# TejasPote/data_diet_distributed

Measured on AMD Instinct MI355X. Metric: examples scored/sec (whole node), EL2N+GraNd ResNet-18 CIFAR-10, 1/2/4/8 GPU, higher is better.
Workload: dtype fp32 (split MFMA: hi*hi + hi*lo + lo*hi with fp32 accumulation; EL2N forward on f16x3 halves, GraNd forward on f16x3, GraNd backward on bf16x3); 1 GPU; R18/C10 EL2N+GraNd, K checkpoints, global keep-set; arch=resnet18, input=3x32x32 cifar stem, n_examples=50000, checkpoints=10, classes=10, score_batch=128, grand_batch=1024, el2n_chunk=1024, kept=25000, select_by=el2n, pegrad_method=auto, grand_params=conv_linear, passes=sequential, lanes=3, launch_plan=full chunks + short tail, el2n_operands=f16x3

## Files before the change

### data_diet_distributed_amd/csrc/dd_pegrad.hip

```cpp
#include "dd_common.h"
#include "dd_mfma.h"
#include "dd_pgram.h"
#include "dd_stem.h"

namespace dd {

typedef float floatx16 __attribute__((ext_vector_type(16)));
typedef float floatx4 __attribute__((ext_vector_type(4)));

struct Geom {
  int cin, h, w, cout, ho, wo, kh, kw, stride, pad;
};

__device__ __forceinline__ unsigned xcd_remap(unsigned orig, unsigned nwg) {
  const unsigned q = nwg / 8, r = nwg % 8, xcd = orig % 8;
  return (xcd < r ? xcd * (q + 1) : r * (q + 1) + (xcd - r) * q) + orig / 8;
}

constexpr int DBM = 64, DBN = 64, DBK = 32;

__global__ __launch_bounds__(256) void pegrad_direct_kernel(const float* __restrict__ act,
                                                            const float* __restrict__ gout,
                                                            Geom g, int n_cblk, int n_oblk,
                                                            const float* __restrict__ col_scale,
                                                            float* __restrict__ partial) {
  __shared__ float As[DBK][DBM + 1];
  __shared__ float Bs[DBK][DBN + 1];
  __shared__ float red[4];

  const int ntiles = g.kh * g.kw * n_cblk * n_oblk;
  const unsigned lid = xcd_remap(blockIdx.x, gridDim.x);
  const int b = lid / ntiles;
  int tile = lid - b * ntiles;
  const int ob = tile % n_oblk;
  tile /= n_oblk;
  const int cb = tile % n_cblk;
  const int shift = tile / n_cblk;
  const int ky = shift / g.kw, kx = shift - (shift / g.kw) * g.kw;
  const int c0 = cb * DBM, o0 = ob * DBN;
  const int T = g.ho * g.wo, HW = g.h * g.w;
  const float* a_b = act + (size_t)b * g.cin * HW;
  const float* g_b = gout + (size_t)b * g.cout * T;

  const int tid = threadIdx.x, tl = tid & 31, rg = tid >> 5;
  float ra[8], rb[8];
  auto load = [&](int t0) {
    const int t = t0 + tl;
    const bool vt = t < T;
    const int oy = vt ? t / g.wo : 0;
    const int ox = vt ? t - oy * g.wo : 0;
    const int iy = oy * g.stride + ky - g.pad, ix = ox * g.stride + kx - g.pad;
    const bool va = vt && iy >= 0 && iy < g.h && ix >= 0 && ix < g.w;
    const int off = iy * g.w + ix;
#pragma unroll
    for (int j = 0; j < 8; ++j) {
      const int c = c0 + rg + 8 * j;
      ra[j] = (va && c < g.cin) ? a_b[(size_t)c * HW + off] : 0.f;
      const int o = o0 + rg + 8 * j;
      rb[j] = (vt && o < g.cout) ? g_b[(size_t)o * T + t] : 0.f;
    }
  };

  const int lane = tid & 63, wv = tid >> 6, wm = wv & 1, wn = wv >> 1;
  const int kr = lane >> 5, col = lane & 31;
  floatx16 acc = {0};
  const int nk = (T + DBK - 1) / DBK;
  load(0);
  for (int kt = 0; kt < nk; ++kt) {
    __syncthreads();
#pragma unroll
    for (int j = 0; j < 8; ++j) {
      As[tl][rg + 8 * j] = ra[j];
      Bs[tl][rg + 8 * j] = rb[j];
    }
    __syncthreads();
    if (kt + 1 < nk) load((kt + 1) * DBK);
#pragma unroll
    for (int kk = 0; kk < DBK / 2; ++kk) {
      const float av = As[2 * kk + kr][wm * 32 + col];
      const float bv = Bs[2 * kk + kr][wn * 32 + col];
      acc = __builtin_amdgcn_mfma_f32_32x32x2f32(av, bv, acc, 0, 0, 0);
    }
  }
  const int o = o0 + wn * 32 + col;
  float s2 = 1.f;
  if (col_scale) {
    const float s = (o < g.cout) ? col_scale[o] : 0.f;
    s2 = s * s;
  }
  float v = 0.f;
#pragma unroll
  for (int r = 0; r < 16; ++r) v += acc[r] * acc[r];
  v = wave_sum(v * s2);
  if (lane == 0) red[wv] = v;
  __syncthreads();
  if (tid == 0) partial[lid] = (red[0] + red[1]) + (red[2] + red[3]);
}

typedef __bf16 bf16x8_t __attribute__((ext_vector_type(8)));
typedef __bf16 bf16x4_t __attribute__((ext_vector_type(4)));

template <int S, int LC>
__global__ __launch_bounds__(256) void pegrad_direct1x1_kernel(const float* __restrict__ act,
                                                               const float* __restrict__ gout,
                                                               Geom g, int n_cblk, int n_oblk,
                                                               const float* __restrict__ col_scale,
                                                               float* __restrict__ partial) {
  constexpr int LO = 4 / LC;
  constexpr int MC = 64 * LC, MO = 64 * LO, R = MC + MO;
  constexpr int KT = 32;
  constexpr int RS = KT * 2 + 16;
  constexpr int PL = R * RS;
  constexpr int NL = R * (KT / 4) / 256;
  static_assert(R * (KT / 4) % 256 == 0, "whole float4 loads per thread");
  __shared__ __attribute__((aligned(16))) char lds[2 * PL];
  __shared__ float red[4];
  const int ntiles = n_cblk * n_oblk;
  const unsigned lid = xcd_remap(blockIdx.x, gridDim.x);
  const int b = lid / ntiles;
  const int tile = lid - b * ntiles;
  const int ob = tile % n_oblk, cb = tile / n_oblk;
  const int c0 = cb * MC, o0 = ob * MO;
  const int T = g.ho * g.wo, HW = g.h * g.w;
  const int tid = threadIdx.x, lane = tid & 63, wv = tid >> 6;
  const float* __restrict__ a_b = act + (size_t)b * g.cin * HW;
  const float* __restrict__ g_b = gout + (size_t)b * g.cout * T;
  const bool vec = T % 4 == 0 && (S == 1 || g.wo % 4 == 0) && HW % 4 == 0;

  float4 rv[NL];
  auto load = [&](int t0) {
#pragma unroll
    for (int k = 0; k < NL; ++k) {
      const int q = tid + 256 * k, row = q / (KT / 4), x4 = q % (KT / 4);
      const int t = t0 + 4 * x4;
      const bool isa = row < MC;
      const int ch = isa ? c0 + row : o0 + row - MC;
      const bool rok = ch < (isa ? g.cin : g.cout);
      const float* base = isa ? a_b + (size_t)(rok ? ch : 0) * HW
                              : g_b + (size_t)(rok ? ch : 0) * T;
      float v[4] = {0.f, 0.f, 0.f, 0.f};
      if (vec) {
        if (rok && t < T) {
          if (!isa || S == 1) {
            const float4 u = *reinterpret_cast<const float4*>(base + t);
            v[0] = u.x; v[1] = u.y; v[2] = u.z; v[3] = u.w;
          } else {
            const int oy = t / g.wo, ox = t - oy * g.wo;
            const float* src = base + (size_t)oy * S * g.w + ox * S;
            const float4 u0 = *reinterpret_cast<const float4*>(src);
            const float4 u1 = *reinterpret_cast<const float4*>(src + 4);
            v[0] = u0.x; v[1] = u0.z; v[2] = u1.x; v[3] = u1.z;
          }
        }
      } else {
#pragma unroll
        for (int j = 0; j < 4; ++j) {
          const int tj = t + j;
          if (rok && tj < T) {
            int ia = tj;
            if (isa && S != 1) {
              const int oy = tj / g.wo, ox = tj - oy * g.wo;
              ia = oy * S * g.w + ox * S;
            }
            v[j] = base[ia];
          }
        }
      }
      rv[k] = make_float4(v[0], v[1], v[2], v[3]);
    }
  };
  auto stage = [&]() {
#pragma unroll
    for (int k = 0; k < NL; ++k) {
      const int q = tid + 256 * k, row = q / (KT / 4), x4 = q % (KT / 4);
      const float f[4] = {rv[k].x, rv[k].y, rv[k].z, rv[k].w};
      bf16x4_t hv, lv;
#pragma unroll
      for (int j = 0; j < 4; ++j) {
        const __bf16 x = (__bf16)f[j];
        hv[j] = x;
        lv[j] = (__bf16)(f[j] - (float)x);
      }
      char* p = lds + row * RS + x4 * 8;
      *reinterpret_cast<bf16x4_t*>(p) = hv;
      *reinterpret_cast<bf16x4_t*>(p + PL) = lv;
    }
  };

  const int r = lane & 31, h = lane >> 5;
  const int wc = wv % LC, wo_ = wv / LC;
  floatx16 acc[2][2];
#pragma unroll
  for (int i = 0; i < 2; ++i)
#pragma unroll
    for (int j = 0; j < 2; ++j) acc[i][j] = floatx16{0};
  load(0);
  for (int t0 = 0; t0 < T; t0 += KT) {
    __syncthreads();
    stage();
    __syncthreads();
    if (t0 + KT < T) load(t0 + KT);
#pragma unroll
    for (int s = 0; s < 2; ++s) {
      bf16x8_t ah[2], al[2], gh[2], gl[2];
#pragma unroll
      for (int i = 0; i < 2; ++i) {
        const char* pa = lds + (wc * 64 + 32 * i + r) * RS + (16 * s + 8 * h) * 2;
        const char* pg = lds + (MC + wo_ * 64 + 32 * i + r) * RS + (16 * s + 8 * h) * 2;
        ah[i] = *reinterpret_cast<const bf16x8_t*>(pa);
        al[i] = *reinterpret_cast<const bf16x8_t*>(pa + PL);
        gh[i] = *reinterpret_cast<const bf16x8_t*>(pg);
        gl[i] = *reinterpret_cast<const bf16x8_t*>(pg + PL);
      }
#pragma unroll
      for (int i = 0; i < 2; ++i)
#pragma unroll
        for (int j = 0; j < 2; ++j) {
          floatx16 d = acc[i][j];
          d = __builtin_amdgcn_mfma_f32_32x32x16_bf16(ah[i], gh[j], d, 0, 0, 0);
          d = __builtin_amdgcn_mfma_f32_32x32x16_bf16(ah[i], gl[j], d, 0, 0, 0);
          d = __builtin_amdgcn_mfma_f32_32x32x16_bf16(al[i], gh[j], d, 0, 0, 0);
          acc[i][j] = d;
        }
    }
  }
  float v = 0.f;
#pragma unroll
  for (int j = 0; j < 2; ++j) {
    const int o = o0 + wo_ * 64 + 32 * j + r;
    float s2 = 1.f;
    if (col_scale) {
      const float sc = o < g.cout ? col_scale[o] : 0.f;
      s2 = sc * sc;
    }
    float q = 0.f;
#pragma unroll
    for (int i = 0; i < 2; ++i)
#pragma unroll
      for (int k = 0; k < 16; ++k) q += acc[i][j][k] * acc[i][j][k];
    v += q * s2;
  }
  v = wave_sum(v);
  if (lane == 0) red[wv] = v;
  __syncthreads();
  if (tid == 0) partial[lid] = (red[0] + red[1]) + (red[2] + red[3]);
}

__global__ __launch_bounds__(256) void pegrad_ghost64_kernel(const float* __restrict__ act,
                                                             const float* __restrict__ gout,
                                                             Geom g, int nT,
                                                             const float* __restrict__ col_scale,
                                                             float* __restrict__ partial) {
  __shared__ float red[4];
  const int ntiles = nT * nT;
  const unsigned lid = xcd_remap(blockIdx.x, gridDim.x);
  const int b = lid / ntiles;
  const int tile = lid - b * ntiles;
  const int bi = tile / nT, bj = tile - (tile / nT) * nT;
  const int T = g.ho * g.wo, HW = g.h * g.w;
  const float* a_b = act + (size_t)b * g.cin * HW;
  const float* g_b = gout + (size_t)b * g.cout * T;

  const int tid = threadIdx.x, lane = tid & 63, wv = tid >> 6;
  const int h = lane >> 5, r = lane & 31;
  const int ti = bi * 64 + (wv & 1) * 32 + r;
  const int tj = bj * 64 + (wv >> 1) * 32 + r;
  const bool vti = ti < T, vtj = tj < T;
  const int oyi = vti ? ti / g.wo : 0, oxi = vti ? ti - oyi * g.wo : 0;
  const int oyj = vtj ? tj / g.wo : 0, oxj = vtj ? tj - oyj * g.wo : 0;

  floatx16 accA = {0}, accG = {0};
  const int npair = (g.cin + 1) / 2;
  for (int ky = 0; ky < g.kh; ++ky) {
    for (int kx = 0; kx < g.kw; ++kx) {
      const int iyi = oyi * g.stride + ky - g.pad, ixi = oxi * g.stride + kx - g.pad;
      const int iyj = oyj * g.stride + ky - g.pad, ixj = oxj * g.stride + kx - g.pad;
      const bool vi = vti && iyi >= 0 && iyi < g.h && ixi >= 0 && ixi < g.w;
      const bool vj = vtj && iyj >= 0 && iyj < g.h && ixj >= 0 && ixj < g.w;
      const float* pi = a_b + (vi ? iyi * g.w + ixi : 0);
      const float* pj = a_b + (vj ? iyj * g.w + ixj : 0);
      int p = 0;
      for (; p + 4 <= npair; p += 4) {
        float ai[4], aj[4];
#pragma unroll
        for (int u = 0; u < 4; ++u) {
          const int c = 2 * (p + u) + h;
          ai[u] = (vi && c < g.cin) ? pi[(size_t)c * HW] : 0.f;
          aj[u] = (vj && c < g.cin) ? pj[(size_t)c * HW] : 0.f;
        }
#pragma unroll
        for (int u = 0; u < 4; ++u)
          accA = __builtin_amdgcn_mfma_f32_32x32x2f32(ai[u], aj[u], accA, 0, 0, 0);
      }
      for (; p < npair; ++p) {
        const int c = 2 * p + h;
        const float ai = (vi && c < g.cin) ? pi[(size_t)c * HW] : 0.f;
        const float aj = (vj && c < g.cin) ? pj[(size_t)c * HW] : 0.f;
        accA = __builtin_amdgcn_mfma_f32_32x32x2f32(ai, aj, accA, 0, 0, 0);
      }
    }
  }
  const int opair = (g.cout + 1) / 2;
  for (int p = 0; p < opair; ++p) {
    const int o = 2 * p + h;
    const bool vo = o < g.cout;
    const float s = (col_scale && vo) ? col_scale[o] : 1.f;
    const float gi = (vti && vo) ? g_b[(size_t)o * T + ti] * s : 0.f;
    const float gj = (vtj && vo) ? g_b[(size_t)o * T + tj] * s : 0.f;
    accG = __builtin_amdgcn_mfma_f32_32x32x2f32(gi, gj, accG, 0, 0, 0);
  }
  float v = 0.f;
#pragma unroll
  for (int k = 0; k < 16; ++k) v += accA[k] * accG[k];
  v = wave_sum(v);
  if (lane == 0) red[wv] = v;
  __syncthreads();
  if (tid == 0) partial[lid] = (red[0] + red[1]) + (red[2] + red[3]);
}

__global__ __launch_bounds__(256) void pegrad_ghost16_kernel(const float* __restrict__ act,
                                                             const float* __restrict__ gout,
                                                             int64_t B, Geom g,
                                                             const float* __restrict__ col_scale,
                                                             float* __restrict__ partial) {
  const int lane = threadIdx.x & 63;
  const int64_t b = (int64_t)blockIdx.x * 4 + (threadIdx.x >> 6);
  if (b >= B) return;
  const int T = g.ho * g.wo, HW = g.h * g.w;
  const float* a_b = act + (size_t)b * g.cin * HW;
  const float* g_b = gout + (size_t)b * g.cout * T;
  const int t = lane & 15, kq = lane >> 4;
  const bool vt = t < T;
  const int oy = vt ? t / g.wo : 0, ox = vt ? t - oy * g.wo : 0;

  floatx4 a0 = {0}, a1 = {0}, gA = {0}, gB = {0};
  const int nq = (g.cin + 3) / 4;
  for (int ky = 0; ky < g.kh; ++ky) {
    for (int kx = 0; kx < g.kw; ++kx) {
      const int iy = oy * g.stride + ky - g.pad, ix = ox * g.stride + kx - g.pad;
      const bool v = vt && iy >= 0 && iy < g.h && ix >= 0 && ix < g.w;
      const float* p = a_b + (v ? iy * g.w + ix : 0);
      int q = 0;
      for (; q + 4 <= nq; q += 4) {
        float x[4];
#pragma unroll
        for (int u = 0; u < 4; ++u) {
          const int c = 4 * (q + u) + kq;
          x[u] = (v && c < g.cin) ? p[(size_t)c * HW] : 0.f;
        }
        a0 = __builtin_amdgcn_mfma_f32_16x16x4f32(x[0], x[0], a0, 0, 0, 0);
        a1 = __builtin_amdgcn_mfma_f32_16x16x4f32(x[1], x[1], a1, 0, 0, 0);
        a0 = __builtin_amdgcn_mfma_f32_16x16x4f32(x[2], x[2], a0, 0, 0, 0);
        a1 = __builtin_amdgcn_mfma_f32_16x16x4f32(x[3], x[3], a1, 0, 0, 0);
      }
      for (; q < nq; ++q) {
        const int c = 4 * q + kq;
        const float x = (v && c < g.cin) ? p[(size_t)c * HW] : 0.f;
        a0 = __builtin_amdgcn_mfma_f32_16x16x4f32(x, x, a0, 0, 0, 0);
      }
    }
  }
  const int no = (g.cout + 3) / 4;
  int q = 0;
  for (; q + 2 <= no; q += 2) {
    float x[2];
#pragma unroll
    for (int u = 0; u < 2; ++u) {
      const int o = 4 * (q + u) + kq;
      const bool vo = o < g.cout;
      const float s = (col_scale && vo) ? col_scale[o] : 1.f;
      x[u] = (vt && vo) ? g_b[(size_t)o * T + t] * s : 0.f;
    }
    gA = __builtin_amdgcn_mfma_f32_16x16x4f32(x[0], x[0], gA, 0, 0, 0);
    gB = __builtin_amdgcn_mfma_f32_16x16x4f32(x[1], x[1], gB, 0, 0, 0);
  }
  for (; q < no; ++q) {
    const int o = 4 * q + kq;
    const bool vo = o < g.cout;
    const float s = (col_scale && vo) ? col_scale[o] : 1.f;
    const float x = (vt && vo) ? g_b[(size_t)o * T + t] * s : 0.f;
    gA = __builtin_amdgcn_mfma_f32_16x16x4f32(x, x, gA, 0, 0, 0);
  }
  float v = 0.f;
#pragma unroll
  for (int k = 0; k < 4; ++k) v += (a0[k] + a1[k]) * (gA[k] + gB[k]);
  v = wave_sum(v);
  if (lane == 0) partial[b] = v;
}

typedef __bf16 bf16x8 __attribute__((ext_vector_type(8)));
typedef __bf16 bf16x4 __attribute__((ext_vector_type(4)));

template <int W, int STR>
struct D3Cfg {
  static constexpr int R = 32 / W;
  static constexpr int NEW = STR * R;
  static constexpr int WIN = STR == 1 ? R + 2 : 2 * R + 1;
  static constexpr int S = WIN + NEW;
  static constexpr int WI = STR * W;
  static constexpr int CS = ((W * 2 / 16) % 2 == 1 || STR == 2) ? W * 2 : W * 2 + 16;
  static constexpr int PLANE = 64 * CS;
  static constexpr int ACT_BYTES = S * 3 * 2 * PLANE;
  static constexpr int GCS = 80;
  static constexpr int GPLANE = 64 * GCS;
  static constexpr int G_BYTES = 2 * 2 * GPLANE;
  static constexpr int LDS = ACT_BYTES + G_BYTES;
  static constexpr int TPR = WI / 4;
  static constexpr int NA = NEW * 64 * WI / 4 / 256;
  static_assert(NEW * 64 * WI / 4 % 256 == 0, "whole float4 rounds");
  static_assert(LDS <= 160 * 1024, "LDS budget");
};

__device__ __forceinline__ void split4(float4 v, bf16x4& hi, bf16x4& lo) {
  const __bf16 h0 = (__bf16)v.x, h1 = (__bf16)v.y, h2 = (__bf16)v.z, h3 = (__bf16)v.w;
  hi = bf16x4{h0, h1, h2, h3};
  lo = bf16x4{(__bf16)(v.x - (float)h0), (__bf16)(v.y - (float)h1), (__bf16)(v.z - (float)h2),
              (__bf16)(v.w - (float)h3)};
}

template <int W, int STR>
__global__ __launch_bounds__(256, 1) void pegrad_direct3x3_kernel(
    const float* __restrict__ act, const float* __restrict__ gout, int cin, int cout, int H,
    int n_cblk, int n_oblk, const float* __restrict__ col_scale, float* __restrict__ partial) {
  using C = D3Cfg<W, STR>;
  extern __shared__ __attribute__((aligned(16))) char smem[];
  char* act_lds = smem;
  char* g_lds = smem + C::ACT_BYTES;

  const unsigned lid = xcd_remap(blockIdx.x, gridDim.x);
  const int per_ex = n_cblk * n_oblk;
  const int b = lid / per_ex;
  const int rem = lid - b * per_ex;
  const int c0 = (rem / n_oblk) * 64, o0 = (rem % n_oblk) * 64;
  const int HW = H * W;
  const int HI = STR * H, HWI = HI * C::WI;
  const float* a_b = act + (size_t)b * cin * HWI;
  const float* g_b = gout + (size_t)b * cout * HW;

  constexpr int NTH = 256;
  const int tid = threadIdx.x, lane = tid & 63, wv = tid >> 6;
  const int wc = wv & 1, wo = (wv >> 1) & 1, r = lane & 31, h = lane >> 5;

  constexpr int NAT = C::NA, NGT = 2;
  float4 ra[NAT], rg[NGT];
  bool va[NAT], vg[NGT];
  auto load_rows = [&](int ir0, int nrows, int tstep) {
#pragma unroll
    for (int k = 0; k < NAT; ++k) {
      const int idx = tid + NTH * k;
      const int x4 = idx % C::TPR, c = (idx / C::TPR) % 64, rr = idx / (C::TPR * 64);
      const int ir = ir0 + rr;
      const int cg = c0 + c;
      va[k] = rr < nrows && ir >= 0 && ir < HI && cg < cin;
      const int irc = ir < 0 ? 0 : (ir >= HI ? HI - 1 : ir);
      const int cgc = cg < cin ? cg : cin - 1;
      ra[k] = *reinterpret_cast<const float4*>(a_b + (size_t)cgc * HWI + irc * C::WI + x4 * 4);
    }
    if (tstep >= 0) {
      const int ts = tstep < HW / 32 ? tstep : HW / 32 - 1;
#pragma unroll
      for (int k = 0; k < NGT; ++k) {
        const int idx = tid + NTH * k;
        const int o = idx >> 3, t4 = idx & 7;
        const int og = o0 + o;
        vg[k] = og < cout;
        const int ogc = og < cout ? og : cout - 1;
        rg[k] = *reinterpret_cast<const float4*>(g_b + (size_t)ogc * HW + ts * 32 + t4 * 4);
      }
    }
  };
  auto zero_if = [](float4 v, bool ok) { return conv::keep_if(v, ok); };
  auto store_rows = [&](int ir0, int nrows, int gbuf) {
#pragma unroll
    for (int k = 0; k < NAT; ++k) {
      const int idx = tid + NTH * k;
      const int x4 = idx % C::TPR, c = (idx / C::TPR) % 64, rr = idx / (C::TPR * 64);
      if (nrows < C::NEW && rr >= nrows) continue;
      const int slot = (ir0 + rr + 1) % C::S;
      const float4 v = zero_if(ra[k], va[k]);
      if constexpr (STR == 1) {
        static_assert(C::TPR <= 16 && 16 % C::TPR == 0, "row of lanes inside a DPP row");
        uint2 hs[3], ls[3];
        conv::split_shift3(v, x4 == 0, x4 == C::TPR - 1, hs, ls);
#pragma unroll
        for (int kx = 0; kx < 3; ++kx) {
          char* base = act_lds + ((slot * 3 + kx) * 2) * C::PLANE + c * C::CS + x4 * 8;
          *reinterpret_cast<uint2*>(base) = hs[kx];
          *reinterpret_cast<uint2*>(base + C::PLANE) = ls[kx];
        }
      } else {
        float left = conv::lane_prev<C::TPR>(v.w);
        if (x4 == 0) left = 0.f;
        const float f[5] = {left, v.x, v.y, v.z, v.w};
        __bf16 hv[5], lv[5];
#pragma unroll
        for (int i = 0; i < 5; ++i) {
          hv[i] = (__bf16)f[i];
          lv[i] = (__bf16)(f[i] - (float)hv[i]);
        }
        typedef __bf16 bf16x2 __attribute__((ext_vector_type(2)));
#pragma unroll
        for (int kx = 0; kx < 3; ++kx) {
          char* base = act_lds + ((slot * 3 + kx) * 2) * C::PLANE + c * C::CS + x4 * 4;
          *reinterpret_cast<bf16x2*>(base) = bf16x2{hv[kx], hv[kx + 2]};
          *reinterpret_cast<bf16x2*>(base + C::PLANE) = bf16x2{lv[kx], lv[kx + 2]};
        }
      }
    }
    if (gbuf >= 0) {
#pragma unroll
      for (int k = 0; k < NGT; ++k) {
        const int idx = tid + NTH * k;
        const int o = idx >> 3, t4 = idx & 7;
        bf16x4 hi, lo;
        split4(zero_if(rg[k], vg[k]), hi, lo);
        char* base = g_lds + ((gbuf * 2) * 64 + o) * C::GCS + t4 * 8;
        *reinterpret_cast<bf16x4*>(base) = hi;
        *reinterpret_cast<bf16x4*>(base + C::GPLANE) = lo;
      }
    }
  };

  constexpr int NTAP = 9;
  floatx16 acc[NTAP];
#pragma unroll
  for (int i = 0; i < NTAP; ++i) acc[i] = floatx16{0};

  const int nsteps = H / C::R;
  for (int ir0 = -1; ir0 < C::WIN - 1; ir0 += C::NEW) {
    const int n = C::NEW < C::WIN - 1 - ir0 ? C::NEW : C::WIN - 1 - ir0;
    load_rows(ir0, n, ir0 == -1 ? 0 : -1);
    store_rows(ir0, n, ir0 == -1 ? 0 : -1);
  }
  __syncthreads();

  auto frag = [&](int y0, int gbuf, int s, int t, int lo) -> bf16x8 {
    const int tl = 16 * s + 8 * h;
    const int ro = tl / W, x = tl % W;
    if (t < 0) {
      const char* gb = g_lds + ((gbuf * 2) * 64 + wo * 32 + r) * C::GCS + tl * 2;
      return *reinterpret_cast<const bf16x8*>(gb + lo * C::GPLANE);
    }
    const int ky = t / 3, kx = t % 3;
    const int slot = (STR * (y0 + ro) + ky) % C::S;
    const char* ab = act_lds + ((slot * 3 + kx) * 2) * C::PLANE + (wc * 32 + r) * C::CS + x * 2;
    return *reinterpret_cast<const bf16x8*>(ab + lo * C::PLANE);
  };
  auto tap_step = [&](int y0, int gbuf, int inext) {
    bf16x8 bh0, bl0, ah0[NTAP], al0[NTAP], bh1, bl1, ah1[NTAP], al1[NTAP];
    bh0 = frag(y0, gbuf, 0, -1, 0);
    bl0 = frag(y0, gbuf, 0, -1, 1);
    ah0[0] = frag(y0, gbuf, 0, 0, 0);
    al0[0] = frag(y0, gbuf, 0, 0, 1);
    auto rd = [&](int j) {
      constexpr int J0 = 2 * (NTAP - 1), J1 = J0 + 2, J2 = J1 + 2 * NTAP;
      if (j < J0) {
        if (j & 1) al0[1 + j / 2] = frag(y0, gbuf, 0, 1 + j / 2, 1);
        else ah0[1 + j / 2] = frag(y0, gbuf, 0, 1 + j / 2, 0);
      } else if (j < J1) {
        (j == J0 ? bh1 : bl1) = frag(y0, gbuf, 1, -1, j - J0);
      } else if (j < J2) {
        if ((j - J1) & 1) al1[(j - J1) / 2] = frag(y0, gbuf, 1, (j - J1) / 2, 1);
        else ah1[(j - J1) / 2] = frag(y0, gbuf, 1, (j - J1) / 2, 0);
      }
    };
#pragma unroll
    for (int i = 0; i < NTAP; ++i) {
#pragma unroll
      for (int q = 0; q < 3; ++q) {
        __builtin_amdgcn_sched_barrier(0);
        acc[i] = __builtin_amdgcn_mfma_f32_32x32x16_bf16(q == 2 ? al0[i] : ah0[i],
                                                         q == 1 ? bl0 : bh0, acc[i], 0, 0, 0);
        const int g = 3 * i + q;
        const int j0 = g < NTAP ? 2 * g : NTAP + g, nr = g < NTAP ? 2 : 1;
        rd(j0);
        if (nr == 2) rd(j0 + 1);
      }
    }
    __builtin_amdgcn_sched_barrier(0);
#pragma unroll
    for (int i = 0; i < NTAP; ++i) {
      floatx16 a = acc[i];
      a = __builtin_amdgcn_mfma_f32_32x32x16_bf16(ah1[i], bh1, a, 0, 0, 0);
      a = __builtin_amdgcn_mfma_f32_32x32x16_bf16(ah1[i], bl1, a, 0, 0, 0);
      a = __builtin_amdgcn_mfma_f32_32x32x16_bf16(al1[i], bh1, a, 0, 0, 0);
      acc[i] = a;
    }
    store_rows(inext, C::NEW, gbuf ^ 1);
#pragma unroll
    for (int i = 0; i < 3 * NTAP - 1; ++i) {
      __builtin_amdgcn_sched_group_barrier(0x008, 1, 1);
      __builtin_amdgcn_sched_group_barrier(0x002, 4, 1);
      __builtin_amdgcn_sched_group_barrier(0x080, 1, 1);
    }
    __builtin_amdgcn_sched_group_barrier(0x008, 1, 1);
    __builtin_amdgcn_sched_barrier(0);
  };
  for (int st = 0; st < nsteps; ++st) {
    const int y0 = st * C::R;
    const int inext = STR * y0 + C::WIN - 1;
    load_rows(inext, C::NEW, st + 1);
    const int gbuf = st & 1;
    tap_step(y0, gbuf, inext);
    __syncthreads();
  }

  const int o = o0 + wo * 32 + r;
  float s2 = (o < cout) ? 1.f : 0.f;
  if (col_scale && o < cout) {
    const float sc = col_scale[o];
    s2 = sc * sc;
  }
  float v = 0.f;
#pragma unroll
  for (int i = 0; i < NTAP; ++i)
#pragma unroll
    for (int k = 0; k < 16; ++k) v += acc[i][k] * acc[i][k];
  v = wave_sum(v * s2);
  float* red = reinterpret_cast<float*>(smem);
  if (lane == 0) red[wv] = v;
  __syncthreads();
  if (tid == 0) partial[lid] = (red[0] + red[1]) + (red[2] + red[3]);
}

template <int W, int STR>
static void launch_direct3x3(const float* act, const float* gout, int64_t B, int cin, int cout,
                             int H, const float* col_scale, float* partial, hipStream_t st) {
  using C = D3Cfg<W, STR>;
  const int ncb = (int)ceil_div(cin, 64), nob = (int)ceil_div(cout, 64);
  static bool attr_set = false;
  if (!attr_set) {
    (void)hipFuncSetAttribute(reinterpret_cast<const void*>(&pegrad_direct3x3_kernel<W, STR>),
                              hipFuncAttributeMaxDynamicSharedMemorySize, C::LDS);
    attr_set = true;
  }
  pegrad_direct3x3_kernel<W, STR><<<(unsigned)(B * ncb * nob), 256, C::LDS, st>>>(
      act, gout, cin, cout, H, ncb, nob, col_scale, partial);
}

template <int W, int STR>
__global__ __launch_bounds__(256, 1) void pegrad_direct3x3p_kernel(
    const float* __restrict__ act, const float* __restrict__ gout, int cin, int cout, int H,
    int n_cblk, int n_oblk, const float* __restrict__ col_scale, float* __restrict__ partial,
    int total) {
  using C = D3Cfg<W, STR>;
  extern __shared__ __attribute__((aligned(16))) char smem[];
  char* act_lds = smem;
  char* g_lds = smem + C::ACT_BYTES;
  float* red = reinterpret_cast<float*>(smem + C::LDS);

  const int per_ex = n_cblk * n_oblk;
  const int HW = H * W;
  const int HI = STR * H, HWI = HI * C::WI;
  int lid, c0, o0;
  const float *a_b, *g_b;
  auto set_tile = [&](int t) {
    lid = (int)xcd_remap((unsigned)t, (unsigned)total);
    const int b = lid / per_ex;
    const int rem = lid - b * per_ex;
    c0 = (rem / n_oblk) * 64;
    o0 = (rem % n_oblk) * 64;
    a_b = act + (size_t)b * cin * HWI;
    g_b = gout + (size_t)b * cout * HW;
  };

  constexpr int NTH = 256;
  const int tid = threadIdx.x, lane = tid & 63, wv = tid >> 6;
  const int wc = wv & 1, wo = (wv >> 1) & 1, r = lane & 31, h = lane >> 5;

  constexpr int NAW = C::WIN * 64 * C::WI / 4 / NTH;
  static_assert(C::WIN * 64 * C::WI / 4 % NTH == 0, "whole float4 rounds");
  constexpr int NGT = 2;
  float4 ra[NAW], rg[NGT];
  bool va[NAW], vg[NGT];
  auto load_rows = [&](auto NKc, int ir0, int nrows, int tstep) {
    constexpr int NK = decltype(NKc)::value;
#pragma unroll
    for (int k = 0; k < NK; ++k) {
      const int idx = tid + NTH * k;
      const int x4 = idx % C::TPR, c = (idx / C::TPR) % 64, rr = idx / (C::TPR * 64);
      const int ir = ir0 + rr;
      const int cg = c0 + c;
      va[k] = rr < nrows && ir >= 0 && ir < HI && cg < cin;
      const int irc = ir < 0 ? 0 : (ir >= HI ? HI - 1 : ir);
      const int cgc = cg < cin ? cg : cin - 1;
      ra[k] = *reinterpret_cast<const float4*>(a_b + (size_t)cgc * HWI + irc * C::WI + x4 * 4);
    }
    if (tstep >= 0) {
      const int ts = tstep < HW / 32 ? tstep : HW / 32 - 1;
#pragma unroll
      for (int k = 0; k < NGT; ++k) {
        const int idx = tid + NTH * k;
        const int o = idx >> 3, t4 = idx & 7;
        const int og = o0 + o;
        vg[k] = og < cout;
        const int ogc = og < cout ? og : cout - 1;
        rg[k] = *reinterpret_cast<const float4*>(g_b + (size_t)ogc * HW + ts * 32 + t4 * 4);
      }
    }
  };
  auto zero_if = [](float4 v, bool ok) { return conv::keep_if(v, ok); };
  auto store_rows = [&](auto NKc, int ir0, int gbuf) {
    constexpr int NK = decltype(NKc)::value;
#pragma unroll
    for (int k = 0; k < NK; ++k) {
      const int idx = tid + NTH * k;
      const int x4 = idx % C::TPR, c = (idx / C::TPR) % 64, rr = idx / (C::TPR * 64);
      const int slot = (ir0 + rr + 1) % C::S;
      const float4 v = zero_if(ra[k], va[k]);
      if constexpr (STR == 1) {
        static_assert(C::TPR <= 16 && 16 % C::TPR == 0, "row of lanes inside a DPP row");
        uint2 hs[3], ls[3];
        conv::split_shift3(v, x4 == 0, x4 == C::TPR - 1, hs, ls);
#pragma unroll
        for (int kx = 0; kx < 3; ++kx) {
          char* base = act_lds + ((slot * 3 + kx) * 2) * C::PLANE + c * C::CS + x4 * 8;
          *reinterpret_cast<uint2*>(base) = hs[kx];
          *reinterpret_cast<uint2*>(base + C::PLANE) = ls[kx];
        }
      } else {
        float left = conv::lane_prev<C::TPR>(v.w);
        if (x4 == 0) left = 0.f;
        const float f[5] = {left, v.x, v.y, v.z, v.w};
        __bf16 hv[5], lv[5];
#pragma unroll
        for (int i = 0; i < 5; ++i) {
          hv[i] = (__bf16)f[i];
          lv[i] = (__bf16)(f[i] - (float)hv[i]);
        }
        typedef __bf16 bf16x2 __attribute__((ext_vector_type(2)));
#pragma unroll
        for (int kx = 0; kx < 3; ++kx) {
          char* base = act_lds + ((slot * 3 + kx) * 2) * C::PLANE + c * C::CS + x4 * 4;
          *reinterpret_cast<bf16x2*>(base) = bf16x2{hv[kx], hv[kx + 2]};
          *reinterpret_cast<bf16x2*>(base + C::PLANE) = bf16x2{lv[kx], lv[kx + 2]};
        }
      }
    }
    if (gbuf >= 0) {
#pragma unroll
      for (int k = 0; k < NGT; ++k) {
        const int idx = tid + NTH * k;
        const int o = idx >> 3, t4 = idx & 7;
        bf16x4 hi, lo;
        split4(zero_if(rg[k], vg[k]), hi, lo);
        char* base = g_lds + ((gbuf * 2) * 64 + o) * C::GCS + t4 * 8;
        *reinterpret_cast<bf16x4*>(base) = hi;
        *reinterpret_cast<bf16x4*>(base + C::GPLANE) = lo;
      }
    }
  };

  constexpr int NTAP = 9;
  floatx16 acc[NTAP];
  const std::integral_constant<int, C::NA> KN;
  const std::integral_constant<int, NAW> KW;

  const int nsteps = H / C::R;
  int t = blockIdx.x;
  set_tile(t);
  load_rows(KW, -1, C::WIN, 0);
  store_rows(KW, -1, 0);
  __syncthreads();

  auto frag = [&](int y0, int gbuf, int s, int t, int lo) -> bf16x8 {
    const int tl = 16 * s + 8 * h;
    const int ro = tl / W, x = tl % W;
    if (t < 0) {
      const char* gb = g_lds + ((gbuf * 2) * 64 + wo * 32 + r) * C::GCS + tl * 2;
      return *reinterpret_cast<const bf16x8*>(gb + lo * C::GPLANE);
    }
    const int ky = t / 3, kx = t % 3;
    const int slot = (STR * (y0 + ro) + ky) % C::S;
    const char* ab = act_lds + ((slot * 3 + kx) * 2) * C::PLANE + (wc * 32 + r) * C::CS + x * 2;
    return *reinterpret_cast<const bf16x8*>(ab + lo * C::PLANE);
  };
  auto step = [&](int st, auto LASTc, bool has_next) {
    constexpr bool LAST = decltype(LASTc)::value;
    const int y0 = st * C::R;
    const int inext = STR * y0 + C::WIN - 1;
    if constexpr (!LAST) {
      load_rows(KN, inext, C::NEW, st + 1);
    } else {
      if (has_next) load_rows(KW, -1, C::WIN, 0);
    }
    const int gbuf = st & 1;
    {
      bf16x8 bh0, bl0, ah0[NTAP], al0[NTAP], bh1, bl1, ah1[NTAP], al1[NTAP];
      bh0 = frag(y0, gbuf, 0, -1, 0);
      bl0 = frag(y0, gbuf, 0, -1, 1);
      ah0[0] = frag(y0, gbuf, 0, 0, 0);
      al0[0] = frag(y0, gbuf, 0, 0, 1);
      auto rd = [&](int j) {
        constexpr int J0 = 2 * (NTAP - 1), J1 = J0 + 2, J2 = J1 + 2 * NTAP;
        if (j < J0) {
          if (j & 1) al0[1 + j / 2] = frag(y0, gbuf, 0, 1 + j / 2, 1);
          else ah0[1 + j / 2] = frag(y0, gbuf, 0, 1 + j / 2, 0);
        } else if (j < J1) {
          (j == J0 ? bh1 : bl1) = frag(y0, gbuf, 1, -1, j - J0);
        } else if (j < J2) {
          if ((j - J1) & 1) al1[(j - J1) / 2] = frag(y0, gbuf, 1, (j - J1) / 2, 1);
          else ah1[(j - J1) / 2] = frag(y0, gbuf, 1, (j - J1) / 2, 0);
        }
      };
#pragma unroll
      for (int i = 0; i < NTAP; ++i) {
#pragma unroll
        for (int q = 0; q < 3; ++q) {
          __builtin_amdgcn_sched_barrier(0);
          acc[i] = __builtin_amdgcn_mfma_f32_32x32x16_bf16(q == 2 ? al0[i] : ah0[i],
                                                           q == 1 ? bl0 : bh0, acc[i], 0, 0, 0);
          const int g = 3 * i + q;
          const int j0 = g < NTAP ? 2 * g : NTAP + g, nr = g < NTAP ? 2 : 1;
          rd(j0);
          if (nr == 2) rd(j0 + 1);
        }
      }
      __builtin_amdgcn_sched_barrier(0);
#pragma unroll
      for (int i = 0; i < NTAP; ++i) {
        floatx16 a = acc[i];
        a = __builtin_amdgcn_mfma_f32_32x32x16_bf16(ah1[i], bh1, a, 0, 0, 0);
        a = __builtin_amdgcn_mfma_f32_32x32x16_bf16(ah1[i], bl1, a, 0, 0, 0);
        a = __builtin_amdgcn_mfma_f32_32x32x16_bf16(al1[i], bh1, a, 0, 0, 0);
        acc[i] = a;
      }
      if constexpr (!LAST) {
        store_rows(KN, inext, gbuf ^ 1);
#pragma unroll
        for (int i = 0; i < 3 * NTAP - 1; ++i) {
          __builtin_amdgcn_sched_group_barrier(0x008, 1, 1);
          __builtin_amdgcn_sched_group_barrier(0x002, 4, 1);
          __builtin_amdgcn_sched_group_barrier(0x080, 1, 1);
        }
        __builtin_amdgcn_sched_group_barrier(0x008, 1, 1);
      }
      __builtin_amdgcn_sched_barrier(0);
    }
    __syncthreads();
  };

  for (;;) {
#pragma unroll
    for (int i = 0; i < NTAP; ++i) acc[i] = floatx16{0};
    for (int st = 0; st + 1 < nsteps; ++st) step(st, std::false_type{}, false);
    const int lid_c = lid, o0_c = o0;
    const int tn = t + (int)gridDim.x;
    const bool has_next = tn < total;
    if (has_next) set_tile(tn);
    step(nsteps - 1, std::true_type{}, has_next);

    const int o = o0_c + wo * 32 + r;
    float s2 = (o < cout) ? 1.f : 0.f;
    if (col_scale && o < cout) {
      const float sc = col_scale[o];
      s2 = sc * sc;
    }
    float v = 0.f;
#pragma unroll
    for (int i = 0; i < NTAP; ++i)
#pragma unroll
      for (int k = 0; k < 16; ++k) v += acc[i][k] * acc[i][k];
    v = wave_sum(v * s2);
    if (lane == 0) red[wv] = v;
    if (has_next) store_rows(KW, -1, 0);
    __syncthreads();
    if (tid == 0) partial[lid_c] = (red[0] + red[1]) + (red[2] + red[3]);
    if (!has_next) break;
    __syncthreads();
    t = tn;
  }
}

template <int W, int STR>
static void launch_direct3x3p(const float* act, const float* gout, int64_t B, int cin, int cout,
                              int H, const float* col_scale, float* partial, hipStream_t st) {
  using C = D3Cfg<W, STR>;
  const int ncb = (int)ceil_div(cin, 64), nob = (int)ceil_div(cout, 64);
  constexpr int LDS = C::LDS + 16;
  static_assert(LDS <= 160 * 1024, "LDS budget");
  static bool attr_set = false;
  if (!attr_set) {
    (void)hipFuncSetAttribute(reinterpret_cast<const void*>(&pegrad_direct3x3p_kernel<W, STR>),
                              hipFuncAttributeMaxDynamicSharedMemorySize, LDS);
    attr_set = true;
  }
  const int64_t total = B * ncb * nob;
  const int64_t grid = std::min<int64_t>(total, device_cus());
  pegrad_direct3x3p_kernel<W, STR><<<(unsigned)grid, 256, LDS, st>>>(
      act, gout, cin, cout, H, ncb, nob, col_scale, partial, (int)total);
}

static bool direct3x3_ok(const dd_conv_geom* g) {
  if (g->kh != 3 || g->kw != 3 || g->pad != 1) return false;
  if (g->stride == 1)
    return g->ho == g->h && g->wo == g->w && (g->w == 8 || g->w == 16 || g->w == 32) &&
           (g->h % (32 / g->w)) == 0;
  return g->stride == 2 && g->h == 2 * g->ho && g->w == 2 * g->wo && g->wo == 16 &&
         (g->ho % 2) == 0;
}

__global__ __launch_bounds__(256) void reduce_partials_kernel(const float* __restrict__ partial,
                                                              int64_t B, int ntiles,
                                                              float* __restrict__ sq) {
  const int64_t b = (int64_t)blockIdx.x * blockDim.x + threadIdx.x;
  if (b >= B) return;
  const float* p = partial + b * ntiles;
  float s = 0.f;
  for (int i = 0; i < ntiles; ++i) s += p[i];
  sq[b] += s;
}

struct Plan {
  int method;
  int ghost16;
  int d3x3;
  int d1x1;
  int pgram;
  int pgq;
  int stem;
  int ntiles;
  int n_cblk, n_oblk, nT;
};

static bool geom_ok(const dd_conv_geom* gm) {
  if (!gm) return false;
  if (gm->batch < 0 || gm->cin <= 0 || gm->cout <= 0 || gm->h <= 0 || gm->w <= 0) return false;
  if (gm->kh <= 0 || gm->kw <= 0 || gm->stride <= 0 || gm->pad < 0) return false;
  const int ho = (gm->h + 2 * gm->pad - gm->kh) / gm->stride + 1;
  const int wo = (gm->w + 2 * gm->pad - gm->kw) / gm->stride + 1;
  return ho == gm->ho && wo == gm->wo && ho > 0 && wo > 0;
}

static double direct_cost(const dd_conv_geom* gm) {
  const double T = (double)ceil_div((int64_t)gm->ho * gm->wo, DBK) * DBK;
  const double da = (double)gm->kh * gm->kw * ceil_div(gm->cin, DBM) * DBM;
  const double dg = (double)ceil_div(gm->cout, DBN) * DBN;
  return 2.0 * T * da * dg;
}

static double ghost_cost(const dd_conv_geom* gm) {
  const int64_t T = (int64_t)gm->ho * gm->wo;
  if (T <= 16) {
    const double da = (double)gm->kh * gm->kw * ceil_div(gm->cin, 4) * 4;
    const double dg = (double)ceil_div(gm->cout, 4) * 4;
    return 2.0 * 256.0 * (da + dg);
  }
  const double Tp = (double)ceil_div(T, 64) * 64;
  const double da = (double)gm->kh * gm->kw * ceil_div(gm->cin, 2) * 2;
  const double dg = (double)ceil_div(gm->cout, 2) * 2;
  return 2.0 * Tp * Tp * (da + dg) * 1.5;
}

static constexpr double kD3x3Weight = 0.25;

static int d1x1_layout(const dd_conv_geom* gm) {
  int best = 0;
  double best_eff = 0.0;
  for (int lc = 1; lc <= 4; lc *= 2) {
    const double pc = (double)ceil_div(gm->cin, 64 * lc) * 64 * lc;
    const double po = (double)ceil_div(gm->cout, 64 * (4 / lc)) * 64 * (4 / lc);
    const double eff = (double)gm->cin * gm->cout / (pc * po);
    if (eff > best_eff + 1e-9) {
      best_eff = eff;
      best = lc;
    }
  }
  return best_eff >= 0.75 ? best : 0;
}

static Plan make_plan(const dd_conv_geom* gm, int method, int precision) {
  Plan p{};
  const bool d3 = precision == DD_PREC_BF16X3 && direct3x3_ok(gm);
  const bool d1 = precision == DD_PREC_BF16X3 && gm->kh == 1 && gm->kw == 1 && gm->pad == 0 &&
                  (gm->stride == 1 || gm->stride == 2) &&
                  gm->ho == (gm->h - 1) / gm->stride + 1 &&
                  gm->wo == (gm->w - 1) / gm->stride + 1 && d1x1_layout(gm) > 0;
  if (precision == DD_PREC_BF16X3 && method != DD_PEGRAD_GHOST && stem_ok(gm)) {
    p.method = DD_PEGRAD_DIRECT;
    p.stem = 1;
    p.ntiles = 1;
    return p;
  }
  if (precision == DD_PREC_BF16X3 && method != DD_PEGRAD_DIRECT && pgram_ok(gm)) {
    p.method = DD_PEGRAD_GHOST;
    p.pgram = 1;
    p.ntiles = 1;
    return p;
  }
  if (precision == DD_PREC_BF16X3 && method != DD_PEGRAD_DIRECT && pgram_q_ok(gm) &&
      (method == DD_PEGRAD_GHOST || pgram_q_auto())) {
    p.method = DD_PEGRAD_GHOST;
    p.pgq = 1;
    p.ntiles = 4;
    return p;
  }
  if (method == DD_PEGRAD_AUTO) {
    const double dc = direct_cost(gm) * (d3 ? kD3x3Weight : 1.0);
    method = ghost_cost(gm) < dc ? DD_PEGRAD_GHOST : DD_PEGRAD_DIRECT;
  }
  p.method = method;
  const int64_t T = (int64_t)gm->ho * gm->wo;
  if (method == DD_PEGRAD_DIRECT && d1) {
    p.d1x1 = d1x1_layout(gm);
    p.n_cblk = (int)ceil_div(gm->cin, 64 * p.d1x1);
    p.n_oblk = (int)ceil_div(gm->cout, 64 * (4 / p.d1x1));
    p.ntiles = p.n_cblk * p.n_oblk;
  } else if (method == DD_PEGRAD_DIRECT && d3) {
    p.d3x3 = 1;
    p.n_cblk = (int)ceil_div(gm->cin, 64);
    p.n_oblk = (int)ceil_div(gm->cout, 64);
    p.ntiles = p.n_cblk * p.n_oblk;
  } else if (method == DD_PEGRAD_DIRECT) {
    p.n_cblk = (int)ceil_div(gm->cin, DBM);
    p.n_oblk = (int)ceil_div(gm->cout, DBN);
    p.ntiles = gm->kh * gm->kw * p.n_cblk * p.n_oblk;
  } else {
    p.ghost16 = T <= 16;
    p.nT = (int)ceil_div(T, 64);
    p.ntiles = p.ghost16 ? 1 : p.nT * p.nT;
  }
  return p;
}

}

using namespace dd;

extern "C" {

static bool prec_ok(int precision) {
  return precision == DD_PREC_FP32 || precision == DD_PREC_BF16X3;
}

int dd_conv_pegrad_method(const dd_conv_geom* geom, int method, int precision) {
  clear_error();
  DD_REQUIRE(geom_ok(geom), "dd_conv_pegrad_method: inconsistent conv geometry");
  DD_REQUIRE(method >= DD_PEGRAD_AUTO && method <= DD_PEGRAD_GHOST, "bad method %d", method);
  DD_REQUIRE(prec_ok(precision), "bad precision %d", precision);
  const Plan p = make_plan(geom, method, precision);
  return p.d3x3 ? DD_PEGRAD_DIRECT3X3 : p.d1x1 ? DD_PEGRAD_DIRECT1X1 : p.pgram ? DD_PEGRAD_PGRAM
         : p.pgq ? DD_PEGRAD_PGRAM_Q : p.stem ? DD_PEGRAD_STEM : p.method;
}

size_t dd_conv_pegrad_workspace_bytes(const dd_conv_geom* geom, int method, int precision) {
  if (!geom_ok(geom) || method < DD_PEGRAD_AUTO || method > DD_PEGRAD_GHOST ||
      !prec_ok(precision))
    return 0;
  const Plan p = make_plan(geom, method, precision);
  return (size_t)geom->batch * p.ntiles * sizeof(float);
}

int dd_conv_pegrad_sqnorm(const float* act, const float* gout, const dd_conv_geom* geom,
                          const float* col_scale, int method, int precision, float* sq_accum,
                          void* workspace, size_t workspace_bytes, void* stream) {
  clear_error();
  DD_REQUIRE(geom_ok(geom), "dd_conv_pegrad_sqnorm: inconsistent conv geometry");
  DD_REQUIRE(method >= DD_PEGRAD_AUTO && method <= DD_PEGRAD_GHOST, "bad method %d", method);
  DD_REQUIRE(prec_ok(precision), "bad precision %d", precision);
  const int64_t B = geom->batch;
  if (B == 0) return DD_OK;
  DD_REQUIRE(act && gout && sq_accum, "dd_conv_pegrad_sqnorm: null buffer");
  DD_REQUIRE((int64_t)geom->cin * geom->h * geom->w < (1ll << 31) &&
                 (int64_t)geom->cout * geom->ho * geom->wo < (1ll << 31),
             "dd_conv_pegrad_sqnorm: per-example tensor too large");
  const Plan p = make_plan(geom, method, precision);
  const size_t need = (size_t)B * p.ntiles * sizeof(float);
  if (workspace_bytes < need || !workspace) {
    set_error("dd_conv_pegrad_sqnorm: workspace %zu < %zu bytes", workspace_bytes, need);
    return DD_EWORKSPACE;
  }
  float* partial = static_cast<float*>(workspace);
  Geom g{geom->cin, geom->h, geom->w, geom->cout, geom->ho, geom->wo,
         geom->kh, geom->kw, geom->stride, geom->pad};
  hipStream_t st = as_stream(stream);
  if (p.pgram) return pgram_launch(act, gout, geom, col_scale, sq_accum, st);
  if (p.stem) return stem_launch(act, gout, geom, col_scale, sq_accum, st);
  const int64_t nblk = B * p.ntiles;
  DD_REQUIRE(nblk < (1ll << 31), "dd_conv_pegrad_sqnorm: grid too large");
  if (p.pgq) {
    pgram_q_launch(act, gout, geom, col_scale, partial, st);
  } else if (p.d3x3) {
    if (geom->stride == 2)
      launch_direct3x3p<16, 2>(act, gout, B, geom->cin, geom->cout, geom->ho, col_scale, partial,
                               st);
    else if (geom->w == 32)
      launch_direct3x3<32, 1>(act, gout, B, geom->cin, geom->cout, geom->h, col_scale, partial,
                              st);
    else if (geom->w == 16)
      launch_direct3x3p<16, 1>(act, gout, B, geom->cin, geom->cout, geom->h, col_scale, partial,
                               st);
    else
      launch_direct3x3<8, 1>(act, gout, B, geom->cin, geom->cout, geom->h, col_scale, partial,
                             st);
  } else if (p.d1x1) {
#define DD_D1(S_, LC_)                                                                   \
  pegrad_direct1x1_kernel<S_, LC_><<<(unsigned)nblk, 256, 0, st>>>(act, gout, g, p.n_cblk, \
                                                                   p.n_oblk, col_scale, partial)
    if (geom->stride == 1) {
      if (p.d1x1 == 1) DD_D1(1, 1); else if (p.d1x1 == 2) DD_D1(1, 2); else DD_D1(1, 4);
    } else {
      if (p.d1x1 == 1) DD_D1(2, 1); else if (p.d1x1 == 2) DD_D1(2, 2); else DD_D1(2, 4);
    }
#undef DD_D1
  } else if (p.method == DD_PEGRAD_DIRECT) {
    pegrad_direct_kernel<<<(unsigned)nblk, 256, 0, st>>>(act, gout, g, p.n_cblk, p.n_oblk,
                                                         col_scale, partial);
  } else if (p.ghost16) {
    pegrad_ghost16_kernel<<<(unsigned)ceil_div(B, 4), 256, 0, st>>>(act, gout, B, g,
                                                                   col_scale, partial);
  } else {
    pegrad_ghost64_kernel<<<(unsigned)nblk, 256, 0, st>>>(act, gout, g, p.nT, col_scale,
                                                          partial);
  }
  DD_CHECK_LAUNCH("dd_conv_pegrad_sqnorm");
  reduce_partials_kernel<<<(unsigned)ceil_div(B, 256), 256, 0, st>>>(partial, B, p.ntiles,
                                                                     sq_accum);
  DD_CHECK_LAUNCH("dd_conv_pegrad_sqnorm(reduce)");
  return DD_OK;
}

}
```

Baseline: 9018 examples/s.

## Keep 3x3 conv activation window resident in registers across row steps

For the 32-wide stride-1 per-example gradient norm kernel, activation MFMA fragments for the three-row window are held in registers and rotated. Each step reads only the one new row from LDS instead of re-reading all nine taps. Steps are unrolled by the window period so register-set indices stay compile-time constants. The gain is less LDS read traffic, paid for with much higher VGPR pressure and possible spills. A new scheduling order interleaves MFMAs with the new-row loads.

```diff
diff --git a/data_diet_distributed_amd/csrc/dd_pegrad.hip b/data_diet_distributed_amd/csrc/dd_pegrad.hip
--- a/data_diet_distributed_amd/csrc/dd_pegrad.hip
+++ b/data_diet_distributed_amd/csrc/dd_pegrad.hip
@@ -418,7 +418,74 @@
               (__bf16)(v.w - (float)h3)};
 }
 
-template <int W, int STR>
+struct D3Win {
+  using C = D3Cfg<32, 1>;
+  static constexpr int PERIOD = 3;
+  static_assert(C::WIN == PERIOD && C::NEW == 1, "one row enters a three-row window per step");
+  static constexpr int set_of(int p, int d) { return (p + d) % C::WIN; }
+  typedef bf16x8 Frags[C::WIN][3][2][2];
+  static __device__ __forceinline__ bf16x8 read(const char* act_lds, int y0, int d, int kx,
+                                                int s, int lo, int arow, int h) {
+    const int slot = (y0 + d) % C::S;
+    return *reinterpret_cast<const bf16x8*>(act_lds + ((slot * 3 + kx) * 2 + lo) * C::PLANE +
+                                            arow * C::CS + (16 * s + 8 * h) * 2);
+  }
+  static __device__ __forceinline__ void fill(Frags& f, const char* act_lds, int arow, int h) {
+    conv::static_for<2 * 12>([&](auto Jc) {
+      constexpr int j = decltype(Jc)::value;
+      constexpr int d = j / 12, s = j / 6 % 2, kx = j % 6 / 2, lo = j & 1;
+      f[set_of(0, d)][kx][s][lo] = read(act_lds, 0, d, kx, s, lo, arow, h);
+    });
+  }
+};
+
+template <int P, typename Stage>
+__device__ __forceinline__ void d3_rowreg_step(D3Win::Frags& f, floatx16 (&acc)[9],
+                                               const char* act_lds, const char* g_lds, int y0,
+                                               int gbuf, int arow, int brow, int h,
+                                               Stage&& stage) {
+  using C = D3Win::C;
+  auto bfrag = [&](int s, int lo) {
+    return *reinterpret_cast<const bf16x8*>(g_lds + ((gbuf * 2 + lo) * 64 + brow) * C::GCS +
+                                            (16 * s + 8 * h) * 2);
+  };
+  bf16x8 b[2][2];
+  b[0][0] = bfrag(0, 0);
+  b[0][1] = bfrag(0, 1);
+  constexpr int NEWSET = D3Win::set_of(P, 2);
+  auto rd = [&](auto Jc) {
+    constexpr int j = decltype(Jc)::value;
+    if constexpr (j >= 6 && j < 8) {
+      b[1][j - 6] = bfrag(1, j - 6);
+    } else {
+      constexpr int e = j < 6 ? j : j - 2;
+      constexpr int s = e / 6, kx = e % 6 / 2, lo = e & 1;
+      f[NEWSET][kx][s][lo] = D3Win::read(act_lds, y0, 2, kx, s, lo, arow, h);
+    }
+  };
+  conv::static_for<27>([&](auto Gc) {
+    constexpr int g = decltype(Gc)::value, i = g / 3, q = g % 3;
+    constexpr int set = D3Win::set_of(P, i / 3), kx = i % 3;
+    __builtin_amdgcn_sched_barrier(0);
+    acc[i] = __builtin_amdgcn_mfma_f32_32x32x16_bf16(f[set][kx][0][q == 2], b[0][q == 1],
+                                                     acc[i], 0, 0, 0);
+    if constexpr (g < 14) rd(Gc);
+  });
+  __builtin_amdgcn_sched_barrier(0);
+  conv::static_for<9>([&](auto Ic) {
+    constexpr int i = decltype(Ic)::value;
+    constexpr int set = D3Win::set_of(P, i / 3), kx = i % 3;
+    floatx16 a = acc[i];
+    a = __builtin_amdgcn_mfma_f32_32x32x16_bf16(f[set][kx][1][0], b[1][0], a, 0, 0, 0);
+    a = __builtin_amdgcn_mfma_f32_32x32x16_bf16(f[set][kx][1][0], b[1][1], a, 0, 0, 0);
+    a = __builtin_amdgcn_mfma_f32_32x32x16_bf16(f[set][kx][1][1], b[1][0], a, 0, 0, 0);
+    acc[i] = a;
+  });
+  stage();
+  __builtin_amdgcn_sched_barrier(0);
+}
+
+template <int W, int STR, bool RR>
 __global__ __launch_bounds__(256, 1) void pegrad_direct3x3_kernel(
     const float* __restrict__ act, const float* __restrict__ gout, int cin, int cout, int H,
     int n_cblk, int n_oblk, const float* __restrict__ col_scale, float* __restrict__ partial) {
@@ -596,13 +663,43 @@
     __builtin_amdgcn_sched_group_barrier(0x008, 1, 1);
     __builtin_amdgcn_sched_barrier(0);
   };
-  for (int st = 0; st < nsteps; ++st) {
-    const int y0 = st * C::R;
-    const int inext = STR * y0 + C::WIN - 1;
-    load_rows(inext, C::NEW, st + 1);
-    const int gbuf = st & 1;
-    tap_step(y0, gbuf, inext);
-    __syncthreads();
+  if constexpr (RR) {
+    static_assert(W == 32 && STR == 1, "the resident window is built for the 32-wide kernel");
+    (void)tap_step;
+    D3Win::Frags fw;
+    const int arow = wc * 32 + r, brow = wo * 32 + r;
+    D3Win::fill(fw, act_lds, arow, h);
+    auto rstep = [&](auto Pc, int st) __attribute__((always_inline)) {
+      const int inext = st + C::WIN - 1;
+      load_rows(inext, C::NEW, st + 1);
+      const int gbuf = st & 1;
+      d3_rowreg_step<decltype(Pc)::value>(fw, acc, act_lds, g_lds, st, gbuf, arow, brow, h, [&] {
+        store_rows(inext, C::NEW, gbuf ^ 1);
+#pragma unroll
+        for (int i = 0; i < 3 * NTAP - 1; ++i) {
+          __builtin_amdgcn_sched_group_barrier(0x008, 1, 1);
+          __builtin_amdgcn_sched_group_barrier(0x002, 4, 1);
+          __builtin_amdgcn_sched_group_barrier(0x080, 1, 1);
+        }
+        __builtin_amdgcn_sched_group_barrier(0x008, 1, 1);
+      });
+      __syncthreads();
+    };
+    int st = 0;
+    for (; st + D3Win::PERIOD <= nsteps; st += D3Win::PERIOD)
+      conv::static_for<D3Win::PERIOD>([&](auto Pc) { rstep(Pc, st + decltype(Pc)::value); });
+    conv::static_for<D3Win::PERIOD - 1>([&](auto Pc) {
+      if (st + decltype(Pc)::value < nsteps) rstep(Pc, st + decltype(Pc)::value);
+    });
+  } else {
+    for (int st = 0; st < nsteps; ++st) {
+      const int y0 = st * C::R;
+      const int inext = STR * y0 + C::WIN - 1;
+      load_rows(inext, C::NEW, st + 1);
+      const int gbuf = st & 1;
+      tap_step(y0, gbuf, inext);
+      __syncthreads();
+    }
   }
 
   const int o = o0 + wo * 32 + r;
@@ -623,20 +720,23 @@
   if (tid == 0) partial[lid] = (red[0] + red[1]) + (red[2] + red[3]);
 }
 
-template <int W, int STR>
+template <int W, int STR, bool RR>
 static void launch_direct3x3(const float* act, const float* gout, int64_t B, int cin, int cout,
                              int H, const float* col_scale, float* partial, hipStream_t st) {
   using C = D3Cfg<W, STR>;
   const int ncb = (int)ceil_div(cin, 64), nob = (int)ceil_div(cout, 64);
   static bool attr_set = false;
   if (!attr_set) {
-    (void)hipFuncSetAttribute(reinterpret_cast<const void*>(&pegrad_direct3x3_kernel<W, STR>),
-                              hipFuncAttributeMaxDynamicSharedMemorySize, C::LDS);
+    (void)hipFuncSetAttribute(
+        reinterpret_cast<const void*>(&pegrad_direct3x3_kernel<W, STR, RR>),
+        hipFuncAttributeMaxDynamicSharedMemorySize, C::LDS);
     attr_set = true;
   }
-  pegrad_direct3x3_kernel<W, STR><<<(unsigned)(B * ncb * nob), 256, C::LDS, st>>>(
+  pegrad_direct3x3_kernel<W, STR, RR><<<(unsigned)(B * ncb * nob), 256, C::LDS, st>>>(
       act, gout, cin, cout, H, ncb, nob, col_scale, partial);
 }
+
+static bool rowreg_on() { return env_int("DD_PEGRAD_ROWREG", 1) != 0; }
 
 template <int W, int STR>
 __global__ __launch_bounds__(256, 1) void pegrad_direct3x3p_kernel(
@@ -1084,15 +1184,18 @@
     if (geom->stride == 2)
       launch_direct3x3p<16, 2>(act, gout, B, geom->cin, geom->cout, geom->ho, col_scale, partial,
                                st);
+    else if (geom->w == 32 && rowreg_on())
+      launch_direct3x3<32, 1, true>(act, gout, B, geom->cin, geom->cout, geom->h, col_scale,
+                                    partial, st);
     else if (geom->w == 32)
-      launch_direct3x3<32, 1>(act, gout, B, geom->cin, geom->cout, geom->h, col_scale, partial,
-                              st);
+      launch_direct3x3<32, 1, false>(act, gout, B, geom->cin, geom->cout, geom->h, col_scale,
+                                     partial, st);
     else if (geom->w == 16)
       launch_direct3x3p<16, 1>(act, gout, B, geom->cin, geom->cout, geom->h, col_scale, partial,
                                st);
     else
-      launch_direct3x3<8, 1>(act, gout, B, geom->cin, geom->cout, geom->h, col_scale, partial,
-                             st);
+      launch_direct3x3<8, 1, false>(act, gout, B, geom->cin, geom->cout, geom->h, col_scale,
+                                    partial, st);
   } else if (p.d1x1) {
 #define DD_D1(S_, LC_)                                                                   \
   pegrad_direct1x1_kernel<S_, LC_><<<(unsigned)nblk, 256, 0, st>>>(act, gout, g, p.n_cblk, \
```

Result: no change. 9049 examples/s, median of 6 (+0.3%).
